# guangkun0818/speech2text

Hardware: AMD Instinct MI355X
Metric: audio-seconds/sec (train step, zipformer pruned-RNN-T) (higher is better)
Workload: dtype f32; 1 GPU; C3 zipformer pruned-RNN-T train step: chunk_size -1, 500 BPE, prune_range 5 (fbank+fwd+bwd+allreduce+ScaledAdam); accumulate_grad_batches=1, gemm_arith=bf16x2/3, per_gpu_batch=64, global_batch=64, labels_per_utt=50, parallelism=dp1

## Files before the change

include/s2t_mi355.h:

```cpp
#ifndef S2T_MI355_H_
#define S2T_MI355_H_

#ifdef __cplusplus
extern "C" {
#endif

int s2t_fbank_f32(const float* pcm, long pcm_stride, const long* num_samples, int batch,
                  const float* window400, const float* twiddle512, const int* mel_off,
                  const int* mel_k0, const float* mel_w, int nnz, int num_mel, float eps,
                  float scale_in, const float* cmvn_mean, const float* cmvn_istd, float* out,
                  int max_frames, long* out_frames, void* stream);

#define S2T_CTC_MAX_LABELS 1023
long s2t_ctc_workspace_floats(int B, int T, int Umax);
int s2t_ctc_loss_fwd_bwd(const float* logits, const long* targets, long tgt_stride,
                         const long* in_len, const long* tgt_len, int B, int T, int V, int Umax,
                         int blank, int zero_infinity, const float* grad_scale, float* workspace,
                         float* loss_per_utt, float* grad_logits, void* stream);

int s2t_fill_f32(float* p, long n, float v, void* stream);
int s2t_rnnt_row_exp(const float* x, long rows, int C, float* probs, float* rowmax, void* stream);
int s2t_rnnt_simple_pxpy(const float* am, const float* lm, const float* am_max,
                         const float* lm_max, const float* nrm, const long* symbols,
                         const long* boundary, int B, int S, int T, int C, int blank, float* px,
// ... 42 lines not shown
                        const float* bypass_scale, const float* g, const float* fm, int B, long rows, int D,
                        float* dx, float* d_orig, float* d_bypass_scale, float* dbias, float* dls,
                        void* stream);
int s2t_biasnorm_bwd(const float* x, const float* bias, const float* scales, const float* g,
                     long rows, int D, float* dx, float* dbias, float* dls, void* stream);
long s2t_balancer_bwd_workspace_floats(void);
int s2t_balancer_bwd(const float* x, long ldx, const float* g, long ldg, long rows, int C,
                     float min_mean, float max_mean, float min_rms, float max_rms,
                     float grad_scale, float* out, long ldo, float* workspace, int parity,
                     float act_off, void* stream);
int s2t_balancer_stats(const float* x, long ldx, long rows, int C, float* stats, void* stream);
int s2t_balancer_apply(const float* x, long ldx, const float* g, long ldg, long rows, int C,
                       float min_mean, float max_mean, float min_rms, float max_rms,
                       float grad_scale, float* out, long ldo, const float* stats, float act_off,
                       void* stream);


int s2t_zipconv_fwd(const float* u, long ld, int gate_off, const unsigned char* mask, int T, int B,
                    int C, int K, int chunk, const float* wc, const float* bc, const float* wk,
                    const float* bk, const float* scale, float* y, void* stream);
int s2t_zipconv_fwd_act(const float* u, long ld, int gate_off, const unsigned char* mask, int T, int B,
                        int C, int K, int chunk, const float* wc, const float* bc, const float* wk,
                        const float* bk, const float* scale, float* y, float* y_act, int act_kind,
                        void* stream);
int s2t_zipconv_bwd(const float* u, long ld, int gate_off, const unsigned char* mask, int T, int B,
                    int C, int K, int chunk, const float* wc, const float* wk, const float* bk,
                    const float* scale, const float* dy, float* du, float* dwc, float* dbc,
                    float* dwk, float* dbk, float* dscale, float* workspace, void* stream);
int s2t_zipconv_bwd_data(const float* u, long ld, int gate_off, const unsigned char* mask, int T,
                         int B, int C, int K, int chunk, const float* wc, const float* wk,
// ... 20 lines not shown
                        int delta_given, float* delta_ws, float* dqkp, float* dpos,
                        float* workspace, void* stream);
long s2t_relpos_attn_bwd_workspace_floats(int T, int B, int H, int pd);
int s2t_attn_apply(const float* W, const float* v, int T, int B, int H, int dv, int transpose,
                   float* out, void* stream);


long s2t_linear_wgrad_workspace_floats(int R, int N, int M);
int s2t_linear_wgrad(const float* g, long ldg, const float* a, long lda, int R, int N, int M,
                     float* dW, float* db, int accumulate, float* workspace, void* stream);

int s2t_whiten_metric(float* xtx, float* colsum, long n, int G, int cg, float* cov, float* mean,
                      float* scal, float* host_metric, float* workspace, void* stream);
int s2t_whiten_prep(const float* cov, const float* mean, const float* scal, int G, int cg, float* dcov,
                    float* bias, float* sums64, void* stream);
int s2t_gemm_x3p_sq(const float* A, long lda, const unsigned short* Bp, int N, int K, float* C, long ldc,
                    int M, const float* bias, const float* other, long ld_other, float* sums, int tile,
                    void* stream);
int s2t_sumsq64(const float* g, long numel, float* sums64, void* stream);
int s2t_whiten_combine64(const float* g, const float* pg, long numel, float grad_scale,
                         const float* sums64, float* out, void* stream);
int s2t_whiten_dcov(const float* cov, const float* mean, const float* scal, int G, int cg,
                    float* dcov, float* bias, float* sums, void* stream);
int s2t_whiten_apply(const float* g, const float* pg, long numel, float grad_scale, float* sums,
                     float* out, void* stream);
int s2t_limit_param_grad(const float* x, const float* g, float lo, float hi, long n, float* out,
                         void* stream);

int s2t_bestrq_labels(const float* feats, int B, int T, int F, const float* proj, int D,
                      const float* codebooks, int ncb, int K, int T2, long* labels, void* stream);
// ... 406 lines not shown
```

speech2text_amd/csrc/gemm_x3p.hip:

```cpp
#include "common.h"
#include "../../include/s2t_mi355.h"
#include <hip/hip_ext.h>
#include <algorithm>
#include <cstdint>
#include <cstdlib>
#include <utility>
#include <vector>

namespace {

typedef float f32x16 __attribute__((ext_vector_type(16)));
typedef float f32x2 __attribute__((ext_vector_type(2)));
typedef __bf16 bf16x2 __attribute__((ext_vector_type(2)));
typedef __bf16 bf16x8 __attribute__((ext_vector_type(8)));
typedef float f32x4 __attribute__((ext_vector_type(4)));
typedef unsigned u32x4 __attribute__((ext_vector_type(4)));
typedef const __attribute__((address_space(1))) float* gf32p;
typedef const __attribute__((address_space(1))) f32x4* gf32x4p;
typedef const __attribute__((address_space(1))) u32x4* gu32x4p;

__device__ __forceinline__ void split_pair(float x0, float x1, unsigned& p0, unsigned& p1,
                                           unsigned& p2) {
  f32x2 x = {x0, x1};
  p0 = __builtin_bit_cast(unsigned, __builtin_convertvector(x, bf16x2));
  f32x2 h = {__uint_as_float(p0 << 16), __uint_as_float(p0 & 0xFFFF0000u)};
  x = x - h;
  p1 = __builtin_bit_cast(unsigned, __builtin_convertvector(x, bf16x2));
  f32x2 h1 = {__uint_as_float(p1 << 16), __uint_as_float(p1 & 0xFFFF0000u)};
  x = x - h1;
  p2 = __builtin_bit_cast(unsigned, __builtin_convertvector(x, bf16x2));
}
__device__ __forceinline__ void split8(const f32x4 v0, const f32x4 v1, u32x4& q0, u32x4& q1,
                                       u32x4& q2) {
  unsigned a0, a1, a2, b0, b1, b2, c0, c1, c2, d0, d1, d2;
  split_pair(v0.x, v0.y, a0, a1, a2);
  split_pair(v0.z, v0.w, b0, b1, b2);
  split_pair(v1.x, v1.y, c0, c1, c2);
  split_pair(v1.z, v1.w, d0, d1, d2);
  q0 = u32x4{a0, b0, c0, d0};
  q1 = u32x4{a1, b1, c1, d1};
  q2 = u32x4{a2, b2, c2, d2};
}

__device__ __forceinline__ void split_pair2(float x0, float x1, unsigned& p0, unsigned& p1) {
  f32x2 x = {x0, x1};
  p0 = __builtin_bit_cast(unsigned, __builtin_convertvector(x, bf16x2));
// ... 138 lines not shown
__device__ __forceinline__ BalQ x3p_epi_balcoef(const X3P& g, int j, int n0, int wcb, int lane) {
  BalQ r;
  r.a = r.b = f32x4{0.f, 0.f, 0.f, 0.f};
  const int col = n0 + 32 * (wcb + j) + (lane & 7) * 4;
  if (col >= g.N) return r;
  r.a = *reinterpret_cast<const f32x4*>(g.bal_stats + 2048 + col);
  r.b = *reinterpret_cast<const f32x4*>(g.bal_stats + 3072 + col);
  return r;
}

__global__ __launch_bounds__(256) void bal_coef_kernel(const float* __restrict__ stats, float* __restrict__ coef,
                                                        int N, float n, float min_mean, float max_mean,
                                                        float min_rms, float max_rms, float gs) {
  const int c = blockIdx.x * 256 + threadIdx.x;
  if (c >= N) return;
  const float inv_n = 1.f / n;
  const float mean = stats[c] * inv_n, uvar = stats[1024 + c] * inv_n;
  const float raw_var = uvar - mean * mean;
  const bool live_v = raw_var > 1.0e-20f, live_r = uvar > 1.0e-20f;
  const float var = fmaxf(raw_var, 1.0e-20f);
  const float sd = sqrtf(var);
  const float rms = sqrtf(fmaxf(uvar, 1.0e-20f));
  const float m = mean / sd;
  const float mc = fminf(fmaxf(m, min_mean), max_mean);
  const float s_m = (m > mc) ? 1.f : ((m < mc) ? -1.f : 0.f);
  const float rc = fminf(fmaxf(rms, min_rms), max_rms);
  const float lq = logf(rc / rms);
  const float s_r = (lq > 0.f) ? -1.f : ((lq < 0.f) ? 1.f : 0.f);
  const float a = s_m * inv_n * (live_v ? (1.f / sd + mean * mean / (sd * var)) : 1.f / sd);
  const float b = (live_v ? -s_m * inv_n * mean / (sd * var) : 0.f) + (live_r ? s_r * inv_n / (rms * rms) : 0.f);
  const float lg_rms = fmaxf(sqrtf(fmaxf(a * a + 2.f * a * b * mean + b * b * uvar, 0.f)), 1.0e-20f);
  const float k = gs / lg_rms;
  coef[c] = a * k;
  coef[1024 + c] = b * k;
}

template <bool BAL = false>
__device__ __forceinline__ void x3p_epi_xform(const X3P& g, f32x16& a, float* scr, const EpiOps& o,
                                              const f32x4 bq, int h, int lane, const BalQ& bal = BalQ{}) {
  const int hi = lane >> 5, lo = lane & 31;
  const int er = lane >> 3, ec = (lane & 7) * 4;
#pragma unroll
  for (int r = 0; r < 8; ++r) scr[((r & 3) + 8 * (r >> 2) + 4 * hi) * 36 + lo] = a[8 * h + r];
  __builtin_amdgcn_fence(__ATOMIC_RELEASE, "workgroup", "local");
  __builtin_amdgcn_wave_barrier();
#pragma unroll
  for (int q = 0; q < 2; ++q) {
    f32x4 v = *reinterpret_cast<const f32x4*>(scr + (er + 8 * q) * 36 + ec);
    v += bq;
// ... 463 lines not shown
}

__global__ __launch_bounds__(256) void x3p_split_kernel(const float* __restrict__ base,
                                                        const S2tPlaneDesc* __restrict__ tab, int n,
                                                        unsigned short* __restrict__ dst) {
  int lo_d = 0, hi_d = n - 1;
  while (lo_d < hi_d) {
    const int mid = (lo_d + hi_d + 1) >> 1;
    if (tab[mid].blk_begin <= blockIdx.x) lo_d = mid; else hi_d = mid - 1;
  }
  const S2tPlaneDesc d = tab[lo_d];
  const int NT = (d.N + 31) >> 5, KB = 2 * ((d.K + 31) >> 5);
  const long q = (long)(blockIdx.x - d.blk_begin) * 4 + (threadIdx.x >> 6);
  if (q >= (long)NT * KB) return;
  const int nt = (int)(q / KB), kb = (int)(q - (long)nt * KB);
  const int lane = threadIdx.x & 63, lo = lane & 31, hi = lane >> 5;
  const int nn = 32 * nt + lo, k0 = 16 * kb + 8 * hi;
  const float* src = base + d.src_off;
  float v[8];
#pragma unroll
  for (int e = 0; e < 8; ++e) {
    const int k = k0 + e;
    const bool ok = nn < d.N && k < d.K;
    const long a = d.transposed ? (long)(ok ? k : 0) * d.ld + (ok ? nn : 0)
                                : (long)(ok ? nn : 0) * d.ld + (ok ? k : 0);
    const float x = src[a];
    v[e] = ok ? x : 0.f;
  }
  uint4 q0, q1, q2;
  split_pair(v[0], v[1], q0.x, q1.x, q2.x);
  split_pair(v[2], v[3], q0.y, q1.y, q2.y);
  split_pair(v[4], v[5], q0.z, q1.z, q2.z);
  split_pair(v[6], v[7], q0.w, q1.w, q2.w);
  unsigned short* o = dst + d.dst_off + (((long)nt * KB + kb) * 3 * 64 + lane) * 8;
  *reinterpret_cast<uint4*>(o) = q0;
  *reinterpret_cast<uint4*>(o + 512) = q1;
  *reinterpret_cast<uint4*>(o + 1024) = q2;
}

#define X3P_LAUNCH(KERNEL, GRID, BLOCK, SMEM)                                                     \
  do {                                                                                            \
    if (s2t_prof_start) {                                                                         \
      hipExtLaunchKernelGGL(KERNEL, dim3(GRID), dim3(BLOCK), SMEM, st, s2t_prof_start,            \
                            s2t_prof_stop, 0, g);                                                 \
      s2t_prof_start = s2t_prof_stop = nullptr;                                                   \
    } else {                                                                                      \
      hipLaunchKernelGGL(KERNEL, dim3(GRID), dim3(BLOCK), SMEM, st, g);                           \
    }                                                                                             \
  } while (0)

template <int TM, int TN, int WPC, int NP = 3, int KS = 1>
void launch_x3p_dma(X3P& g, hipStream_t st) {
// ... 404 lines not shown
```

speech2text_amd/csrc/whiten.hip:

```cpp
#include "common.h"
#include <algorithm>
#include <cstdint>

namespace {

constexpr int NT = 1024;

__device__ __forceinline__ float block_sum(float v, float* s_tmp) {
  v = wave_sum(v);
  const int lane = threadIdx.x & 63, wave = threadIdx.x >> 6;
  __syncthreads();
  if (lane == 0) s_tmp[wave] = v;
  __syncthreads();
  float t = (threadIdx.x < (NT >> 6)) ? s_tmp[threadIdx.x] : 0.f;
  if (wave == 0) {
    t = wave_sum(t);
    if (lane == 0) s_tmp[0] = t;
  }
  __syncthreads();
  return s_tmp[0];
}

__global__ __launch_bounds__(256) void whiten_metric_kernel(float* __restrict__ xtx,
                                                            float* __restrict__ colsum, float n,
// ... 101 lines not shown
    dcov[(long)ci * C + cj] = v;
    acc = fmaf(mean[cj], v, acc);
  }
  acc = wave_sum(acc);
  if ((threadIdx.x & 63) == 0) s_red[threadIdx.x >> 6] = acc;
  __syncthreads();
  if (threadIdx.x == 0) {
    bias[ci] = -((s_red[0] + s_red[1]) + (s_red[2] + s_red[3]));
    if (ci == 0) {
      sums[0] = 0.f;
      sums[1] = 0.f;
    }
  }
}

__global__ __launch_bounds__(256) void sumsq2_kernel(const float* __restrict__ a,
                                                     const float* __restrict__ b, long n,
                                                     float* __restrict__ sums) {
  __shared__ float s_a[4], s_b[4];
  float sa = 0.f, sb = 0.f;
  const long n4 = n >> 2;
  const float4* a4 = reinterpret_cast<const float4*>(a);
  const float4* b4 = reinterpret_cast<const float4*>(b);
  for (long e = (long)blockIdx.x * 256 + threadIdx.x; e < n4; e += (long)gridDim.x * 256) {
    const float4 x = a4[e], y = b4[e];
    sa += x.x * x.x + x.y * x.y + x.z * x.z + x.w * x.w;
    sb += y.x * y.x + y.y * y.y + y.z * y.z + y.w * y.w;
  }
  if (blockIdx.x == 0)
    for (long e = (n4 << 2) + threadIdx.x; e < n; e += 256) {
// ... 87 lines not shown
                     mean, scal, G, cg, dcov, bias, sums);
  S2T_CHECK_LAUNCH();
  return 0;
}

extern "C" int s2t_whiten_prep(const float* cov, const float* mean, const float* scal, int G, int cg,
                               float* dcov, float* bias, float* sums64, void* stream) {
  if (G <= 0 || cg <= 0 || !sums64) return -1;
  if (hipMemsetAsync(sums64, 0, 128 * sizeof(float), (hipStream_t)stream) != hipSuccess) return -3;
  hipLaunchKernelGGL(whiten_dcov_kernel, dim3(G * cg), dim3(256), 0, (hipStream_t)stream, cov, mean,
                     scal, G, cg, dcov, bias, sums64);
  S2T_CHECK_LAUNCH();
  return 0;
}

namespace {
__global__ __launch_bounds__(256) void sumsq64_kernel(const float* __restrict__ g, long numel,
                                                      float* __restrict__ sums64) {
  const long n4 = numel >> 2;
  const long stride = (long)gridDim.x * blockDim.x;
  const float4* g4 = reinterpret_cast<const float4*>(g);
  float acc = 0.f;
  for (long i = (long)blockIdx.x * blockDim.x + threadIdx.x; i < n4; i += stride) {
    const float4 v = g4[i];
    acc += (v.x * v.x + v.y * v.y) + (v.z * v.z + v.w * v.w);
  }
  for (long i = (n4 << 2) + (long)blockIdx.x * blockDim.x + threadIdx.x; i < numel; i += stride) acc += g[i] * g[i];
  acc = wave_sum(acc);
  if ((threadIdx.x & 63) == 0) atomicAdd(sums64 + ((blockIdx.x * 4 + (threadIdx.x >> 6)) & 63), acc);
}
// ... 67 lines not shown
```

speech2text_amd/csrc/zip_elem.hip:

```cpp
#include "common.h"
#include <algorithm>
#include <stdlib.h>

namespace {

__device__ __forceinline__ float log1p_fast(float e) {
  const float u = 1.f + e;
  return u == 1.f ? e : __logf(u) * __fdividef(e, u - 1.f);
}

__device__ __forceinline__ float swoosh_f(float x, float off, float c) {
  const float z = x - off;
  return fmaxf(z, 0.f) + log1p_fast(__expf(-fabsf(z))) - 0.08f * x - c;
}
__device__ __forceinline__ float swoosh_d(float x, float off) {
  return __fdividef(1.f, 1.f + __expf(off - x)) - 0.08f;
}

__global__ __launch_bounds__(256) void swoosh_fwd_kernel(const float* __restrict__ x,
                                                         float* __restrict__ y, long n, float off,
                                                         float c) {
  const long n4 = n >> 2;
  const long stride = (long)gridDim.x * blockDim.x;
  const float4* x4 = reinterpret_cast<const float4*>(x);
// ... 491 lines not shown
  __syncthreads();
  if (threadIdx.x < C) {
    const int c = threadIdx.x;
    const float* f0 = reinterpret_cast<const float*>(&sh[0][0][0]);
    const float* f1 = reinterpret_cast<const float*>(&sh[1][0][0]);
    atomicAdd(&sum[c], (f0[c] + f0[32 + c]) + (f0[64 + c] + f0[96 + c]));
    atomicAdd(&sumsq[c], (f1[c] + f1[32 + c]) + (f1[64 + c] + f1[96 + c]));
  }
}

__global__ __launch_bounds__(256) void balancer_apply_small_kernel(
    const float* __restrict__ x, const float* __restrict__ g, const float* __restrict__ stats,
    float* __restrict__ stats_next, float n, float min_mean, float max_mean, float min_rms, float max_rms,
    float grad_scale, long nquads, int C, float* __restrict__ out, float act_off) {
  __shared__ __attribute__((aligned(16))) float s_a[32], s_b[32];
  const float inv_n = 1.f / n;
  if (threadIdx.x < C) {
    const int c = threadIdx.x;
    const float mean = stats[c] * inv_n, uvar = stats[1024 + c] * inv_n;
    const float raw_var = uvar - mean * mean;
    const bool live_v = raw_var > 1.0e-20f, live_r = uvar > 1.0e-20f;
    const float var = fmaxf(raw_var, 1.0e-20f);
    const float sd = sqrtf(var);
    const float rms = sqrtf(fmaxf(uvar, 1.0e-20f));
    const float m = mean / sd;
    const float mc = fminf(fmaxf(m, min_mean), max_mean);
    const float s_m = (m > mc) ? 1.f : ((m < mc) ? -1.f : 0.f);
    const float rc = fminf(fmaxf(rms, min_rms), max_rms);
    const float lq = logf(rc / rms);
    const float s_r = (lq > 0.f) ? -1.f : ((lq < 0.f) ? 1.f : 0.f);
    const float a = s_m * inv_n * (live_v ? (1.f / sd + mean * mean / (sd * var)) : 1.f / sd);
    const float b = (live_v ? -s_m * inv_n * mean / (sd * var) : 0.f) +
                    (live_r ? s_r * inv_n / (rms * rms) : 0.f);
    const float lg_rms =
        fmaxf(sqrtf(fmaxf(a * a + 2.f * a * b * mean + b * b * uvar, 0.f)), 1.0e-20f);
    const float coef = grad_scale / lg_rms;
    s_a[c] = a * coef;
    s_b[c] = b * coef;
  }
  if (blockIdx.x == 0 && stats_next != nullptr)
    for (int c = threadIdx.x; c < 2 * 1024; c += 256) stats_next[c] = 0.f;
  __syncthreads();
  const int cq = C >> 2;
  const float4 a4 = *reinterpret_cast<const float4*>(&s_a[4 * (threadIdx.x & (cq - 1))]);
  const float4 b4 = *reinterpret_cast<const float4*>(&s_b[4 * (threadIdx.x & (cq - 1))]);
  const float4* x4 = reinterpret_cast<const float4*>(x);
  const float4* g4 = reinterpret_cast<const float4*>(g);
  float4* o4 = reinterpret_cast<float4*>(out);
  const long step = (long)gridDim.x * 256;
  for (long i = (long)blockIdx.x * 256 + threadIdx.x; i < nquads; i += 2 * step) {
    const bool two = i + step < nquads;
    float4 xv[2], gv[2];
    xv[0] = x4[i];
// ... 12 lines not shown
      }
      o4[i + u * step] = make_float4(gg.x + fabsf(gg.x) * fmaf(b4.x, xv[u].x, a4.x),
                                     gg.y + fabsf(gg.y) * fmaf(b4.y, xv[u].y, a4.y),
                                     gg.z + fabsf(gg.z) * fmaf(b4.z, xv[u].z, a4.z),
                                     gg.w + fabsf(gg.w) * fmaf(b4.w, xv[u].w, a4.w));
    }
  }
}

__global__ __launch_bounds__(256) void balancer_apply_fused_kernel(
    const float* __restrict__ x, long ldx, const float* __restrict__ g, long ldg,
    const float* __restrict__ stats, float* __restrict__ stats_next, float n, float min_mean,
    float max_mean, float min_rms, float max_rms, float grad_scale, long rows, int C,
    float* __restrict__ out, long ldo, float act_off) {
  __shared__ float s_a[1024], s_b[1024];
  const float inv_n = 1.f / n;
  for (int c = threadIdx.x; c < C; c += 256) {
    const float mean = stats[c] * inv_n, uvar = stats[1024 + c] * inv_n;
    const float raw_var = uvar - mean * mean;
    const bool live_v = raw_var > 1.0e-20f, live_r = uvar > 1.0e-20f;
    const float var = fmaxf(raw_var, 1.0e-20f);
    const float sd = sqrtf(var);
    const float rms = sqrtf(fmaxf(uvar, 1.0e-20f));
    const float m = mean / sd;
    const float mc = fminf(fmaxf(m, min_mean), max_mean);
    const float s_m = (m > mc) ? 1.f : ((m < mc) ? -1.f : 0.f);
    const float rc = fminf(fmaxf(rms, min_rms), max_rms);
    const float lq = logf(rc / rms);
    const float s_r = (lq > 0.f) ? -1.f : ((lq < 0.f) ? 1.f : 0.f);
    const float a = s_m * inv_n * (live_v ? (1.f / sd + mean * mean / (sd * var)) : 1.f / sd);
    const float b = (live_v ? -s_m * inv_n * mean / (sd * var) : 0.f) +
                    (live_r ? s_r * inv_n / (rms * rms) : 0.f);
    const float lg_rms =
        fmaxf(sqrtf(fmaxf(a * a + 2.f * a * b * mean + b * b * uvar, 0.f)), 1.0e-20f);
    const float coef = grad_scale / lg_rms;
    s_a[c] = a * coef;
    s_b[c] = b * coef;
  }
  if (blockIdx.x == 0 && stats_next != nullptr)
    for (int c = threadIdx.x; c < 2 * 1024; c += 256) stats_next[c] = 0.f;
  __syncthreads();
  const int tx = threadIdx.x & 63, ty = threadIdx.x >> 6;
  const long step = (long)gridDim.x * 4;
  for (int c0 = 0; c0 < C; c0 += 64) {
    const int c = c0 + tx;
    if (c >= C) continue;
    const float a = s_a[c], b = s_b[c];
    long r = (long)blockIdx.x * 4 + ty;
    for (; r + 3 * step < rows; r += 4 * step) {
      float gv[4], xv[4];
#pragma unroll
      for (int u = 0; u < 4; ++u) {
        gv[u] = g[(r + u * step) * ldg + c];
        xv[u] = x[(r + u * step) * ldx + c];
      }
#pragma unroll
      for (int u = 0; u < 4; ++u) {
        if (act_off >= 0.f) gv[u] *= swoosh_d(xv[u], act_off);
        out[(r + u * step) * ldo + c] = gv[u] + fabsf(gv[u]) * fmaf(b, xv[u], a);
      }
    }
    for (; r < rows; r += step) {
// ... 239 lines not shown
  if (bal_small(C, x, ldx, g, ldg, out, ldo)) {
    const long nq = rows * C / 4;
    hipLaunchKernelGGL(balancer_apply_small_kernel, dim3(bal_small_grid(nq)), dim3(256), 0, (hipStream_t)stream,
                       x, g, stats, (float*)nullptr, (float)rows, min_mean, max_mean, min_rms, max_rms, grad_scale,
                       nq, C, out, act_off);
    S2T_CHECK_LAUNCH();
    return 0;
  }
  hipLaunchKernelGGL(balancer_apply_fused_kernel, dim3((unsigned)std::min<long>((rows + 15) / 16, 2048)),
                     dim3(256), 0, (hipStream_t)stream, x, ldx, g, ldg, stats, (float*)nullptr,
                     (float)rows, min_mean, max_mean, min_rms, max_rms, grad_scale, rows, C, out, ldo,
                     act_off);
  S2T_CHECK_LAUNCH();
  return 0;
}
```

Baseline: 17950 audio-seconds/sec.

## Fuse balancer stats with coefficient computation and add one-pass whiten finish kernel

Adds a balancer stats kernel that reduces column sums with a last-block ticket and computes the per-channel balancer coefficients in the same launch, so the apply kernel only reads precomputed coefficients. Adds a whiten_finish kernel that builds the covariance, reduces the metric, computes the bias and splits the whitening matrix into bf16x3 pieces in one launch instead of several. Shared helpers (coefficient math, x3p fragment split) move into headers. The new entry points are only used if the Python side calls them, which is not shown, and the ticket-based grid reduction adds cross-block synchronization risk.

After: 17560 audio-seconds/sec. -2.1%, worse.

```diff
diff --git a/include/s2t_mi355.h b/include/s2t_mi355.h
--- a/include/s2t_mi355.h
+++ b/include/s2t_mi355.h
@@ -80,6 +80,12 @@
                        float min_mean, float max_mean, float min_rms, float max_rms,
                        float grad_scale, float* out, long ldo, const float* stats, float act_off,
                        void* stream);
+long s2t_balancer_stats_ws_floats(void);
+int s2t_balancer_stats_coef(const float* x, long ldx, long rows, int C, float min_mean, float max_mean,
+                            float min_rms, float max_rms, float grad_scale, float* stats, float* workspace,
+                            void* stream);
+int s2t_balancer_apply_coef(const float* x, long ldx, const float* g, long ldg, long rows, int C, float* out,
+                            long ldo, const float* stats, float act_off, void* stream);
 
 
 int s2t_zipconv_fwd(const float* u, long ld, int gate_off, const unsigned char* mask, int T, int B,
@@ -130,6 +136,9 @@
                       float* scal, float* host_metric, float* workspace, void* stream);
 int s2t_whiten_prep(const float* cov, const float* mean, const float* scal, int G, int cg, float* dcov,
                     float* bias, float* sums64, void* stream);
+int s2t_whiten_finish(float* xtx, float* colsum, long n, int G, int cg, float* cov, float* mean, float* scal,
+                      float* host_metric, float* workspace, float* bias, float* sums64, const void* tab,
+                      unsigned short* pieces, void* stream);
 int s2t_gemm_x3p_sq(const float* A, long lda, const unsigned short* Bp, int N, int K, float* C, long ldc,
                     int M, const float* bias, const float* other, long ld_other, float* sums, int tile,
                     void* stream);
diff --git a/speech2text_amd/csrc/balancer_coef.h b/speech2text_amd/csrc/balancer_coef.h
--- /dev/null
+++ b/speech2text_amd/csrc/balancer_coef.h
@@ -0,0 +1,26 @@
+#pragma once
+#include <hip/hip_runtime.h>
+
+__device__ __forceinline__ void s2t_bal_coef_of(float sum, float sumsq, float n, float min_mean, float max_mean,
+                                                float min_rms, float max_rms, float gs, float& ak, float& bk) {
+#pragma clang fp contract(off)
+  const float inv_n = 1.f / n;
+  const float mean = sum * inv_n, uvar = sumsq * inv_n;
+  const float raw_var = uvar - mean * mean;
+  const bool live_v = raw_var > 1.0e-20f, live_r = uvar > 1.0e-20f;
+  const float var = fmaxf(raw_var, 1.0e-20f);
+  const float sd = sqrtf(var);
+  const float rms = sqrtf(fmaxf(uvar, 1.0e-20f));
+  const float m = mean / sd;
+  const float mc = fminf(fmaxf(m, min_mean), max_mean);
+  const float s_m = (m > mc) ? 1.f : ((m < mc) ? -1.f : 0.f);
+  const float rc = fminf(fmaxf(rms, min_rms), max_rms);
+  const float lq = logf(rc / rms);
+  const float s_r = (lq > 0.f) ? -1.f : ((lq < 0.f) ? 1.f : 0.f);
+  const float a = s_m * inv_n * (live_v ? (1.f / sd + mean * mean / (sd * var)) : 1.f / sd);
+  const float b = (live_v ? -s_m * inv_n * mean / (sd * var) : 0.f) + (live_r ? s_r * inv_n / (rms * rms) : 0.f);
+  const float lg_rms = fmaxf(sqrtf(fmaxf(a * a + 2.f * a * b * mean + b * b * uvar, 0.f)), 1.0e-20f);
+  const float k = gs / lg_rms;
+  ak = a * k;
+  bk = b * k;
+}
diff --git a/speech2text_amd/csrc/gemm_x3p.hip b/speech2text_amd/csrc/gemm_x3p.hip
--- a/speech2text_amd/csrc/gemm_x3p.hip
+++ b/speech2text_amd/csrc/gemm_x3p.hip
@@ -1,5 +1,7 @@
 #include "common.h"
 #include "../../include/s2t_mi355.h"
+#include "x3p_split.h"
+#include "balancer_coef.h"
 #include <hip/hip_ext.h>
 #include <algorithm>
 #include <cstdint>
@@ -19,17 +21,6 @@
 typedef const __attribute__((address_space(1))) f32x4* gf32x4p;
 typedef const __attribute__((address_space(1))) u32x4* gu32x4p;
 
-__device__ __forceinline__ void split_pair(float x0, float x1, unsigned& p0, unsigned& p1,
-                                           unsigned& p2) {
-  f32x2 x = {x0, x1};
-  p0 = __builtin_bit_cast(unsigned, __builtin_convertvector(x, bf16x2));
-  f32x2 h = {__uint_as_float(p0 << 16), __uint_as_float(p0 & 0xFFFF0000u)};
-  x = x - h;
-  p1 = __builtin_bit_cast(unsigned, __builtin_convertvector(x, bf16x2));
-  f32x2 h1 = {__uint_as_float(p1 << 16), __uint_as_float(p1 & 0xFFFF0000u)};
-  x = x - h1;
-  p2 = __builtin_bit_cast(unsigned, __builtin_convertvector(x, bf16x2));
-}
 __device__ __forceinline__ void split8(const f32x4 v0, const f32x4 v1, u32x4& q0, u32x4& q1,
                                        u32x4& q2) {
   unsigned a0, a1, a2, b0, b1, b2, c0, c1, c2, d0, d1, d2;
@@ -198,25 +189,7 @@
                                                         float min_rms, float max_rms, float gs) {
   const int c = blockIdx.x * 256 + threadIdx.x;
   if (c >= N) return;
-  const float inv_n = 1.f / n;
-  const float mean = stats[c] * inv_n, uvar = stats[1024 + c] * inv_n;
-  const float raw_var = uvar - mean * mean;
-  const bool live_v = raw_var > 1.0e-20f, live_r = uvar > 1.0e-20f;
-  const float var = fmaxf(raw_var, 1.0e-20f);
-  const float sd = sqrtf(var);
-  const float rms = sqrtf(fmaxf(uvar, 1.0e-20f));
-  const float m = mean / sd;
-  const float mc = fminf(fmaxf(m, min_mean), max_mean);
-  const float s_m = (m > mc) ? 1.f : ((m < mc) ? -1.f : 0.f);
-  const float rc = fminf(fmaxf(rms, min_rms), max_rms);
-  const float lq = logf(rc / rms);
-  const float s_r = (lq > 0.f) ? -1.f : ((lq < 0.f) ? 1.f : 0.f);
-  const float a = s_m * inv_n * (live_v ? (1.f / sd + mean * mean / (sd * var)) : 1.f / sd);
-  const float b = (live_v ? -s_m * inv_n * mean / (sd * var) : 0.f) + (live_r ? s_r * inv_n / (rms * rms) : 0.f);
-  const float lg_rms = fmaxf(sqrtf(fmaxf(a * a + 2.f * a * b * mean + b * b * uvar, 0.f)), 1.0e-20f);
-  const float k = gs / lg_rms;
-  coef[c] = a * k;
-  coef[1024 + c] = b * k;
+  s2t_bal_coef_of(stats[c], stats[1024 + c], n, min_mean, max_mean, min_rms, max_rms, gs, coef[c], coef[1024 + c]);
 }
 
 template <bool BAL = false>
@@ -710,28 +683,10 @@
   const long q = (long)(blockIdx.x - d.blk_begin) * 4 + (threadIdx.x >> 6);
   if (q >= (long)NT * KB) return;
   const int nt = (int)(q / KB), kb = (int)(q - (long)nt * KB);
-  const int lane = threadIdx.x & 63, lo = lane & 31, hi = lane >> 5;
-  const int nn = 32 * nt + lo, k0 = 16 * kb + 8 * hi;
   const float* src = base + d.src_off;
-  float v[8];
-#pragma unroll
-  for (int e = 0; e < 8; ++e) {
-    const int k = k0 + e;
-    const bool ok = nn < d.N && k < d.K;
-    const long a = d.transposed ? (long)(ok ? k : 0) * d.ld + (ok ? nn : 0)
-                                : (long)(ok ? nn : 0) * d.ld + (ok ? k : 0);
-    const float x = src[a];
-    v[e] = ok ? x : 0.f;
-  }
-  uint4 q0, q1, q2;
-  split_pair(v[0], v[1], q0.x, q1.x, q2.x);
-  split_pair(v[2], v[3], q0.y, q1.y, q2.y);
-  split_pair(v[4], v[5], q0.z, q1.z, q2.z);
-  split_pair(v[6], v[7], q0.w, q1.w, q2.w);
-  unsigned short* o = dst + d.dst_off + (((long)nt * KB + kb) * 3 * 64 + lane) * 8;
-  *reinterpret_cast<uint4*>(o) = q0;
-  *reinterpret_cast<uint4*>(o + 512) = q1;
-  *reinterpret_cast<uint4*>(o + 1024) = q2;
+  x3p_split_fragment(d.N, d.K, nt, kb, threadIdx.x & 63, dst + d.dst_off, [&](int nn, int k) {
+    return src[d.transposed ? (long)k * d.ld + nn : (long)nn * d.ld + k];
+  });
 }
 
 #define X3P_LAUNCH(KERNEL, GRID, BLOCK, SMEM)                                                     \
diff --git a/speech2text_amd/csrc/whiten.hip b/speech2text_amd/csrc/whiten.hip
--- a/speech2text_amd/csrc/whiten.hip
+++ b/speech2text_amd/csrc/whiten.hip
@@ -1,4 +1,5 @@
 #include "common.h"
+#include "x3p_split.h"
 #include <algorithm>
 #include <cstdint>
 
@@ -139,6 +140,155 @@
   }
 }
 
+__device__ __forceinline__ void xw_store(float* p, float v) {
+  __hip_atomic_store(p, v, __ATOMIC_RELAXED, __HIP_MEMORY_SCOPE_AGENT);
+}
+__device__ __forceinline__ float xw_load(const float* p) {
+  return __hip_atomic_load(p, __ATOMIC_RELAXED, __HIP_MEMORY_SCOPE_AGENT);
+}
+__device__ __forceinline__ void xw_stores_done() { asm volatile("s_waitcnt vmcnt(0)" ::: "memory"); }
+__global__ __launch_bounds__(1024) void whiten_finish_kernel(float* __restrict__ xtx, float* __restrict__ colsum,
+                                                             float n, int G, int cg, float* cov,
+                                                             float* __restrict__ mean, float* __restrict__ scal,
+                                                             float* host_metric, float* __restrict__ ws,
+                                                             float* __restrict__ bias, float* __restrict__ sums64,
+                                                             const S2tPlaneDesc* __restrict__ desc,
+                                                             unsigned short* __restrict__ pieces) {
+  __shared__ float s_red[2][4];
+  __shared__ unsigned s_old;
+  __shared__ float s_sc[4];
+  __shared__ float s_mean[1024];
+  const int C = G * cg;
+  const int ci = blockIdx.x;
+  const int g = ci / cg, i = ci - g * cg;
+  const float inv_n = 1.f / n;
+  float dsum = 0.f, sq = 0.f;
+  float* xrow = xtx + (long)ci * C;
+  if (threadIdx.x < 256) {
+    const float mi = colsum[ci] * inv_n;
+    for (int j = threadIdx.x; j < cg; j += 256) {
+      const int cj = g * cg + j;
+      if ((cj >> 6) < (ci >> 6)) continue;
+      const float v = xrow[cj] - mi * colsum[cj];
+      xw_store(cov + ((long)g * cg + i) * cg + j, v);
+      sq = fmaf(v, v, sq);
+      if (i == j) dsum = v;
+      if ((cj >> 6) > (ci >> 6)) {
+        xw_store(cov + ((long)g * cg + j) * cg + i, v);
+        sq = fmaf(v, v, sq);
+      }
+    }
+    xw_stores_done();
+  }
+  __syncthreads();
+  for (int j = threadIdx.x; j < C; j += 1024) xrow[j] = 0.f;
+  if (threadIdx.x < 256) {
+    dsum = wave_sum(dsum);
+    sq = wave_sum(sq);
+    if ((threadIdx.x & 63) == 0) {
+      s_red[0][threadIdx.x >> 6] = dsum;
+      s_red[1][threadIdx.x >> 6] = sq;
+    }
+  }
+  __syncthreads();
+  unsigned* ticket = reinterpret_cast<unsigned*>(ws);
+  float* part = ws + 4;
+  if (threadIdx.x == 0) {
+    xw_store(part + 2 * ci, (s_red[0][0] + s_red[0][1]) + (s_red[0][2] + s_red[0][3]));
+    xw_store(part + 2 * ci + 1, (s_red[1][0] + s_red[1][1]) + (s_red[1][2] + s_red[1][3]));
+    xw_stores_done();
+    s_old = atomicAdd(ticket, 1u);
+  }
+  __syncthreads();
+  if (s_old != gridDim.x - 1) return;
+  __builtin_amdgcn_fence(__ATOMIC_ACQUIRE, "agent");
+  if (threadIdx.x < 256) {
+    dsum = 0.f;
+    sq = 0.f;
+    for (int r = threadIdx.x; r < C; r += 256) {
+      dsum += xw_load(part + 2 * r);
+      sq += xw_load(part + 2 * r + 1);
+      const float m = colsum[r] * inv_n;
+      mean[r] = m;
+      s_mean[r] = m;
+    }
+    dsum = wave_sum(dsum);
+    sq = wave_sum(sq);
+  }
+  __syncthreads();
+  if (threadIdx.x < 256 && (threadIdx.x & 63) == 0) {
+    s_red[0][threadIdx.x >> 6] = dsum;
+    s_red[1][threadIdx.x >> 6] = sq;
+  }
+  __syncthreads();
+  for (int r = threadIdx.x; r < C; r += 1024) colsum[r] = 0.f;
+  if (threadIdx.x == 0) {
+    const float dtot = (s_red[0][0] + s_red[0][1]) + (s_red[0][2] + s_red[0][3]);
+    const float sqtot = (s_red[1][0] + s_red[1][1]) + (s_red[1][2] + s_red[1][3]);
+    const float md = dtot / (float)C;
+    const float covsq = sqtot / (float)C;
+    const float denom = md * md + 1.0e-20f;
+    const float metric = covsq / denom;
+    scal[0] = md;
+    scal[1] = covsq;
+    scal[2] = denom;
+    scal[3] = metric;
+    s_sc[0] = md;
+    s_sc[1] = covsq;
+    s_sc[2] = denom;
+    *ticket = 0u;
+    if (host_metric)
+      __hip_atomic_store(host_metric, metric, __ATOMIC_RELAXED, __HIP_MEMORY_SCOPE_SYSTEM);
+  }
+  if (pieces == nullptr) return;
+  if (threadIdx.x < 128) sums64[threadIdx.x] = 0.f;
+  __syncthreads();
+  const float md = s_sc[0], covsq = s_sc[1], denom = s_sc[2];
+  const float k = 4.f / (float)C;
+  const float a = 1.f / denom, d = covsq * md / (denom * denom);
+  const int lane = threadIdx.x & 63, wave = threadIdx.x >> 6;
+#pragma unroll 4
+  for (int r = wave; r < C; r += 16) {
+    const int gr = r / cg;
+    const float* crow = cov + (long)r * cg - (long)gr * cg;
+    float acc[4] = {0.f, 0.f, 0.f, 0.f};
+    const int lo = gr * cg, hi = lo + cg;
+    for (int base = (lo >> 8) << 8; base < hi; base += 256) {
+#pragma unroll
+      for (int w = 0; w < 4; ++w) {
+        const int cj = base + 64 * w + lane;
+        if (cj >= lo && cj < hi) {
+          float v = crow[cj] * a;
+          if (r == cj) v -= d;
+          v *= k;
+          acc[w] = fmaf(s_mean[cj], v, acc[w]);
+        }
+      }
+    }
+#pragma unroll
+    for (int w = 0; w < 4; ++w) acc[w] = wave_sum(acc[w]);
+    if (lane == 0) bias[r] = -((acc[0] + acc[1]) + (acc[2] + acc[3]));
+  }
+  const S2tPlaneDesc ds = desc[0];
+  const int KB = x3p_frag_kb(ds.K);
+  const int nfrag = x3p_frag_nt(ds.N) * KB;
+#pragma unroll 2
+  for (int f = wave; f < nfrag; f += 16) {
+    const int nt = f / KB, kb = f - nt * KB;
+    x3p_split_fragment(ds.N, ds.K, nt, kb, lane, pieces + ds.dst_off, [&](int nn, int kk) {
+      const int r = ds.transposed ? kk : nn, c = ds.transposed ? nn : kk;
+      const int gr = r / cg;
+      float v = 0.f;
+      if (c / cg == gr) {
+        v = cov[(long)r * cg + (c - gr * cg)] * a;
+        if (r == c) v -= d;
+        v *= k;
+      }
+      return v;
+    });
+  }
+}
+
 __global__ __launch_bounds__(256) void sumsq2_kernel(const float* __restrict__ a,
                                                      const float* __restrict__ b, long n,
                                                      float* __restrict__ sums) {
@@ -256,6 +406,18 @@
   return 0;
 }
 
+extern "C" int s2t_whiten_finish(float* xtx, float* colsum, long n, int G, int cg, float* cov, float* mean,
+                                 float* scal, float* host_metric, float* workspace, float* bias,
+                                 float* sums64, const void* tab, unsigned short* pieces, void* stream) {
+  if (G <= 0 || cg <= 0 || n <= 0 || !workspace || (long)G * cg > 1024) return -1;
+  if (pieces && (!bias || !sums64 || !tab || (reinterpret_cast<uintptr_t>(pieces) & 15))) return -1;
+  hipLaunchKernelGGL(whiten_finish_kernel, dim3(G * cg), dim3(1024), 0, (hipStream_t)stream, xtx, colsum,
+                     (float)n, G, cg, cov, mean, scal, host_metric, workspace, bias, sums64,
+                     reinterpret_cast<const S2tPlaneDesc*>(tab), pieces);
+  S2T_CHECK_LAUNCH();
+  return 0;
+}
+
 namespace {
 __global__ __launch_bounds__(256) void sumsq64_kernel(const float* __restrict__ g, long numel,
                                                       float* __restrict__ sums64) {
diff --git a/speech2text_amd/csrc/x3p_split.h b/speech2text_amd/csrc/x3p_split.h
--- /dev/null
+++ b/speech2text_amd/csrc/x3p_split.h
@@ -0,0 +1,50 @@
+#pragma once
+#include "../../include/s2t_mi355.h"
+#include "common.h"
+
+namespace {
+
+typedef float x3ps_f32x2 __attribute__((ext_vector_type(2)));
+typedef __bf16 x3ps_bf16x2 __attribute__((ext_vector_type(2)));
+
+__device__ __forceinline__ void split_pair(float x0, float x1, unsigned& p0, unsigned& p1,
+                                           unsigned& p2) {
+  x3ps_f32x2 x = {x0, x1};
+  p0 = __builtin_bit_cast(unsigned, __builtin_convertvector(x, x3ps_bf16x2));
+  x3ps_f32x2 h = {__uint_as_float(p0 << 16), __uint_as_float(p0 & 0xFFFF0000u)};
+  x = x - h;
+  p1 = __builtin_bit_cast(unsigned, __builtin_convertvector(x, x3ps_bf16x2));
+  x3ps_f32x2 h1 = {__uint_as_float(p1 << 16), __uint_as_float(p1 & 0xFFFF0000u)};
+  x = x - h1;
+  p2 = __builtin_bit_cast(unsigned, __builtin_convertvector(x, x3ps_bf16x2));
+}
+
+__device__ __forceinline__ int x3p_frag_kb(int K) { return 2 * ((K + 31) >> 5); }
+__device__ __forceinline__ int x3p_frag_nt(int N) { return (N + 31) >> 5; }
+
+template <class Load>
+__device__ __forceinline__ void x3p_split_fragment(int N, int K, int nt, int kb, int lane,
+                                                   unsigned short* __restrict__ plane, Load&& load) {
+  const int KB = x3p_frag_kb(K);
+  const int lo = lane & 31, hi = lane >> 5;
+  const int nn = 32 * nt + lo, k0 = 16 * kb + 8 * hi;
+  float v[8];
+#pragma unroll
+  for (int e = 0; e < 8; ++e) {
+    const int k = k0 + e;
+    const bool ok = nn < N && k < K;
+    const float x = load(ok ? nn : 0, ok ? k : 0);
+    v[e] = ok ? x : 0.f;
+  }
+  uint4 q0, q1, q2;
+  split_pair(v[0], v[1], q0.x, q1.x, q2.x);
+  split_pair(v[2], v[3], q0.y, q1.y, q2.y);
+  split_pair(v[4], v[5], q0.z, q1.z, q2.z);
+  split_pair(v[6], v[7], q0.w, q1.w, q2.w);
+  unsigned short* o = plane + (((long)nt * KB + kb) * 3 * 64 + lane) * 8;
+  *reinterpret_cast<uint4*>(o) = q0;
+  *reinterpret_cast<uint4*>(o + 512) = q1;
+  *reinterpret_cast<uint4*>(o + 1024) = q2;
+}
+
+}
diff --git a/speech2text_amd/csrc/zip_elem.hip b/speech2text_amd/csrc/zip_elem.hip
--- a/speech2text_amd/csrc/zip_elem.hip
+++ b/speech2text_amd/csrc/zip_elem.hip
@@ -1,5 +1,8 @@
 #include "common.h"
+#include "balancer_coef.h"
 #include <algorithm>
+#include <cstdint>
+#include <mutex>
 #include <stdlib.h>
 
 namespace {
@@ -529,29 +532,9 @@
     float* __restrict__ stats_next, float n, float min_mean, float max_mean, float min_rms, float max_rms,
     float grad_scale, long nquads, int C, float* __restrict__ out, float act_off) {
   __shared__ __attribute__((aligned(16))) float s_a[32], s_b[32];
-  const float inv_n = 1.f / n;
   if (threadIdx.x < C) {
     const int c = threadIdx.x;
-    const float mean = stats[c] * inv_n, uvar = stats[1024 + c] * inv_n;
-    const float raw_var = uvar - mean * mean;
-    const bool live_v = raw_var > 1.0e-20f, live_r = uvar > 1.0e-20f;
-    const float var = fmaxf(raw_var, 1.0e-20f);
-    const float sd = sqrtf(var);
-    const float rms = sqrtf(fmaxf(uvar, 1.0e-20f));
-    const float m = mean / sd;
-    const float mc = fminf(fmaxf(m, min_mean), max_mean);
-    const float s_m = (m > mc) ? 1.f : ((m < mc) ? -1.f : 0.f);
-    const float rc = fminf(fmaxf(rms, min_rms), max_rms);
-    const float lq = logf(rc / rms);
-    const float s_r = (lq > 0.f) ? -1.f : ((lq < 0.f) ? 1.f : 0.f);
-    const float a = s_m * inv_n * (live_v ? (1.f / sd + mean * mean / (sd * var)) : 1.f / sd);
-    const float b = (live_v ? -s_m * inv_n * mean / (sd * var) : 0.f) +
-                    (live_r ? s_r * inv_n / (rms * rms) : 0.f);
-    const float lg_rms =
-        fmaxf(sqrtf(fmaxf(a * a + 2.f * a * b * mean + b * b * uvar, 0.f)), 1.0e-20f);
-    const float coef = grad_scale / lg_rms;
-    s_a[c] = a * coef;
-    s_b[c] = b * coef;
+    s2t_bal_coef_of(stats[c], stats[1024 + c], n, min_mean, max_mean, min_rms, max_rms, grad_scale, s_a[c], s_b[c]);
   }
   if (blockIdx.x == 0 && stats_next != nullptr)
     for (int c = threadIdx.x; c < 2 * 1024; c += 256) stats_next[c] = 0.f;
@@ -594,29 +577,8 @@
     float max_mean, float min_rms, float max_rms, float grad_scale, long rows, int C,
     float* __restrict__ out, long ldo, float act_off) {
   __shared__ float s_a[1024], s_b[1024];
-  const float inv_n = 1.f / n;
-  for (int c = threadIdx.x; c < C; c += 256) {
-    const float mean = stats[c] * inv_n, uvar = stats[1024 + c] * inv_n;
-    const float raw_var = uvar - mean * mean;
-    const bool live_v = raw_var > 1.0e-20f, live_r = uvar > 1.0e-20f;
-    const float var = fmaxf(raw_var, 1.0e-20f);
-    const float sd = sqrtf(var);
-    const float rms = sqrtf(fmaxf(uvar, 1.0e-20f));
-    const float m = mean / sd;
-    const float mc = fminf(fmaxf(m, min_mean), max_mean);
-    const float s_m = (m > mc) ? 1.f : ((m < mc) ? -1.f : 0.f);
-    const float rc = fminf(fmaxf(rms, min_rms), max_rms);
-    const float lq = logf(rc / rms);
-    const float s_r = (lq > 0.f) ? -1.f : ((lq < 0.f) ? 1.f : 0.f);
-    const float a = s_m * inv_n * (live_v ? (1.f / sd + mean * mean / (sd * var)) : 1.f / sd);
-    const float b = (live_v ? -s_m * inv_n * mean / (sd * var) : 0.f) +
-                    (live_r ? s_r * inv_n / (rms * rms) : 0.f);
-    const float lg_rms =
-        fmaxf(sqrtf(fmaxf(a * a + 2.f * a * b * mean + b * b * uvar, 0.f)), 1.0e-20f);
-    const float coef = grad_scale / lg_rms;
-    s_a[c] = a * coef;
-    s_b[c] = b * coef;
-  }
+  for (int c = threadIdx.x; c < C; c += 256)
+    s2t_bal_coef_of(stats[c], stats[1024 + c], n, min_mean, max_mean, min_rms, max_rms, grad_scale, s_a[c], s_b[c]);
   if (blockIdx.x == 0 && stats_next != nullptr)
     for (int c = threadIdx.x; c < 2 * 1024; c += 256) stats_next[c] = 0.f;
   __syncthreads();
@@ -626,6 +588,287 @@
     const int c = c0 + tx;
     if (c >= C) continue;
     const float a = s_a[c], b = s_b[c];
+    long r = (long)blockIdx.x * 4 + ty;
+    for (; r + 3 * step < rows; r += 4 * step) {
+      float gv[4], xv[4];
+#pragma unroll
+      for (int u = 0; u < 4; ++u) {
+        gv[u] = g[(r + u * step) * ldg + c];
+        xv[u] = x[(r + u * step) * ldx + c];
+      }
+#pragma unroll
+      for (int u = 0; u < 4; ++u) {
+        if (act_off >= 0.f) gv[u] *= swoosh_d(xv[u], act_off);
+        out[(r + u * step) * ldo + c] = gv[u] + fabsf(gv[u]) * fmaf(b, xv[u], a);
+      }
+    }
+    for (; r < rows; r += step) {
+      const float xs = x[r * ldx + c];
+      float gv = g[r * ldg + c];
+      if (act_off >= 0.f) gv *= swoosh_d(xs, act_off);
+      out[r * ldo + c] = gv + fabsf(gv) * fmaf(b, xs, a);
+    }
+  }
+}
+
+
+__device__ __forceinline__ void part_store(float* p, float v) {
+  __hip_atomic_store(p, v, __ATOMIC_RELAXED, __HIP_MEMORY_SCOPE_AGENT);
+}
+__device__ __forceinline__ float part_load(const float* p) {
+  return __hip_atomic_load(p, __ATOMIC_RELAXED, __HIP_MEMORY_SCOPE_AGENT);
+}
+__device__ __forceinline__ void stores_done() { asm volatile("s_waitcnt vmcnt(0)" ::: "memory"); }
+
+struct BalCoefArgs {
+  float n, min_mean, max_mean, min_rms, max_rms, gs;
+};
+
+__global__ __launch_bounds__(256) void col_stats_ticket_kernel(const float* __restrict__ x, long rows, int C,
+                                                               long ld, float* __restrict__ stats,
+                                                               float* part, unsigned* ticket,
+                                                               BalCoefArgs k) {
+  const int c = blockIdx.y * 64 + threadIdx.x;
+  const int Cp = gridDim.y * 64;
+  float s = 0.f, q = 0.f;
+  if (c < C) {
+    const long step = (long)gridDim.x * 4;
+    long r = (long)blockIdx.x * 4 + threadIdx.y;
+    for (; r + 7 * step < rows; r += 8 * step) {
+      float v[8];
+#pragma unroll
+      for (int u = 0; u < 8; ++u) v[u] = x[(r + u * step) * ld + c];
+#pragma unroll
+      for (int u = 0; u < 8; ++u) {
+        s += v[u];
+        q = fmaf(v[u], v[u], q);
+      }
+    }
+    for (; r < rows; r += step) {
+      const float v = x[r * ld + c];
+      s += v;
+      q = fmaf(v, v, q);
+    }
+  }
+  __shared__ float sh[2][4][64];
+  __shared__ unsigned s_old;
+  sh[0][threadIdx.y][threadIdx.x] = s;
+  sh[1][threadIdx.y][threadIdx.x] = q;
+  __syncthreads();
+  if (threadIdx.y == 0) {
+    s = sh[0][0][threadIdx.x] + sh[0][1][threadIdx.x] + sh[0][2][threadIdx.x] + sh[0][3][threadIdx.x];
+    q = sh[1][0][threadIdx.x] + sh[1][1][threadIdx.x] + sh[1][2][threadIdx.x] + sh[1][3][threadIdx.x];
+    float* p = part + (long)blockIdx.x * 2 * Cp;
+    part_store(p + c, s);
+    part_store(p + Cp + c, q);
+    stores_done();
+  }
+  __syncthreads();
+  if (threadIdx.x == 0 && threadIdx.y == 0) s_old = atomicAdd(ticket + blockIdx.y, 1u);
+  __syncthreads();
+  if (s_old != gridDim.x - 1) return;
+  s = 0.f;
+  q = 0.f;
+  {
+    const int nb = (int)gridDim.x;
+    int b = threadIdx.y;
+    for (; b + 124 < nb; b += 128) {
+      float v[32], w[32];
+#pragma unroll
+      for (int u = 0; u < 32; ++u) {
+        v[u] = part_load(part + (long)(b + 4 * u) * 2 * Cp + c);
+        w[u] = part_load(part + (long)(b + 4 * u) * 2 * Cp + Cp + c);
+      }
+#pragma unroll
+      for (int u = 0; u < 32; ++u) {
+        s += v[u];
+        q += w[u];
+      }
+    }
+    for (; b + 28 < nb; b += 32) {
+      float v[8], w[8];
+#pragma unroll
+      for (int u = 0; u < 8; ++u) {
+        v[u] = part_load(part + (long)(b + 4 * u) * 2 * Cp + c);
+        w[u] = part_load(part + (long)(b + 4 * u) * 2 * Cp + Cp + c);
+      }
+#pragma unroll
+      for (int u = 0; u < 8; ++u) {
+        s += v[u];
+        q += w[u];
+      }
+    }
+    for (; b < nb; b += 4) {
+      s += part_load(part + (long)b * 2 * Cp + c);
+      q += part_load(part + (long)b * 2 * Cp + Cp + c);
+    }
+  }
+  __syncthreads();
+  sh[0][threadIdx.y][threadIdx.x] = s;
+  sh[1][threadIdx.y][threadIdx.x] = q;
+  __syncthreads();
+  if (threadIdx.y == 0 && c < C) {
+    s = sh[0][0][threadIdx.x] + sh[0][1][threadIdx.x] + sh[0][2][threadIdx.x] + sh[0][3][threadIdx.x];
+    q = sh[1][0][threadIdx.x] + sh[1][1][threadIdx.x] + sh[1][2][threadIdx.x] + sh[1][3][threadIdx.x];
+    stats[c] = s;
+    stats[1024 + c] = q;
+    float ak, bk;
+    s2t_bal_coef_of(s, q, k.n, k.min_mean, k.max_mean, k.min_rms, k.max_rms, k.gs, ak, bk);
+    stats[2048 + c] = ak;
+    stats[3072 + c] = bk;
+  }
+  if (threadIdx.x == 0 && threadIdx.y == 0) ticket[blockIdx.y] = 0u;
+}
+
+__global__ __launch_bounds__(256) void col_stats_small_ticket_kernel(const float* __restrict__ x, long nquads,
+                                                                     int C, float* __restrict__ stats,
+                                                                     float* part, unsigned* ticket,
+                                                                     BalCoefArgs k) {
+  const int cq = C >> 2;
+  float4 s = make_float4(0.f, 0.f, 0.f, 0.f), q = s;
+  const float4* x4 = reinterpret_cast<const float4*>(x);
+  const long step = (long)gridDim.x * 256;
+  long i = (long)blockIdx.x * 256 + threadIdx.x;
+  for (; i + 3 * step < nquads; i += 4 * step) {
+    float4 v[4];
+#pragma unroll
+    for (int u = 0; u < 4; ++u) v[u] = x4[i + u * step];
+#pragma unroll
+    for (int u = 0; u < 4; ++u) {
+      s.x += v[u].x; s.y += v[u].y; s.z += v[u].z; s.w += v[u].w;
+      q.x = fmaf(v[u].x, v[u].x, q.x); q.y = fmaf(v[u].y, v[u].y, q.y);
+      q.z = fmaf(v[u].z, v[u].z, q.z); q.w = fmaf(v[u].w, v[u].w, q.w);
+    }
+  }
+  for (; i < nquads; i += step) {
+    const float4 v = x4[i];
+    s.x += v.x; s.y += v.y; s.z += v.z; s.w += v.w;
+    q.x = fmaf(v.x, v.x, q.x); q.y = fmaf(v.y, v.y, q.y); q.z = fmaf(v.z, v.z, q.z); q.w = fmaf(v.w, v.w, q.w);
+  }
+  __shared__ float4 sh[2][4][8];
+  __shared__ unsigned s_old;
+  const int lane = threadIdx.x & 63, wave = threadIdx.x >> 6;
+  const float* f0 = reinterpret_cast<const float*>(&sh[0][0][0]);
+  const float* f1 = reinterpret_cast<const float*>(&sh[1][0][0]);
+#pragma unroll
+  for (int o = 32; o >= 1; o >>= 1) {
+    if (o >= cq) {
+      s.x += __shfl_xor(s.x, o, 64); s.y += __shfl_xor(s.y, o, 64);
+      s.z += __shfl_xor(s.z, o, 64); s.w += __shfl_xor(s.w, o, 64);
+      q.x += __shfl_xor(q.x, o, 64); q.y += __shfl_xor(q.y, o, 64);
+      q.z += __shfl_xor(q.z, o, 64); q.w += __shfl_xor(q.w, o, 64);
+    }
+  }
+  if (lane < cq) {
+    sh[0][wave][lane] = s;
+    sh[1][wave][lane] = q;
+  }
+  __syncthreads();
+  float* psum = part;
+  float* psq = part + (long)gridDim.x * C;
+  if (threadIdx.x < C) {
+    const int c = threadIdx.x;
+    part_store(psum + (long)blockIdx.x * C + c, (f0[c] + f0[32 + c]) + (f0[64 + c] + f0[96 + c]));
+    part_store(psq + (long)blockIdx.x * C + c, (f1[c] + f1[32 + c]) + (f1[64 + c] + f1[96 + c]));
+    stores_done();
+  }
+  __syncthreads();
+  if (threadIdx.x == 0) s_old = atomicAdd(ticket, 1u);
+  __syncthreads();
+  if (s_old != gridDim.x - 1) return;
+  float ts = 0.f, tq = 0.f;
+  const long pn = (long)gridDim.x * C;
+  long j = threadIdx.x;
+  for (; j + 7 * 256 < pn; j += 8 * 256) {
+    float v[8], w[8];
+#pragma unroll
+    for (int u = 0; u < 8; ++u) {
+      v[u] = part_load(psum + j + u * 256);
+      w[u] = part_load(psq + j + u * 256);
+    }
+#pragma unroll
+    for (int u = 0; u < 8; ++u) {
+      ts += v[u];
+      tq += w[u];
+    }
+  }
+  for (; j < pn; j += 256) {
+    ts += part_load(psum + j);
+    tq += part_load(psq + j);
+  }
+#pragma unroll
+  for (int o = 32; o >= 4; o >>= 1) {
+    if (o >= C) {
+      ts += __shfl_xor(ts, o, 64);
+      tq += __shfl_xor(tq, o, 64);
+    }
+  }
+  __syncthreads();
+  float* r0 = reinterpret_cast<float*>(&sh[0][0][0]);
+  float* r1 = reinterpret_cast<float*>(&sh[1][0][0]);
+  if (lane < C) {
+    r0[32 * wave + lane] = ts;
+    r1[32 * wave + lane] = tq;
+  }
+  __syncthreads();
+  if (threadIdx.x < C) {
+    const int c = threadIdx.x;
+    ts = (r0[c] + r0[32 + c]) + (r0[64 + c] + r0[96 + c]);
+    tq = (r1[c] + r1[32 + c]) + (r1[64 + c] + r1[96 + c]);
+    stats[c] = ts;
+    stats[1024 + c] = tq;
+    float ak, bk;
+    s2t_bal_coef_of(ts, tq, k.n, k.min_mean, k.max_mean, k.min_rms, k.max_rms, k.gs, ak, bk);
+    stats[2048 + c] = ak;
+    stats[3072 + c] = bk;
+  }
+  if (threadIdx.x == 0) *ticket = 0u;
+}
+
+__global__ __launch_bounds__(256) void balancer_apply_coef_small_kernel(
+    const float* __restrict__ x, const float* __restrict__ g, const float* __restrict__ coef, long nquads, int C,
+    float* __restrict__ out, float act_off) {
+  const int cq = C >> 2;
+  const float4 a4 = *reinterpret_cast<const float4*>(coef + 4 * (threadIdx.x & (cq - 1)));
+  const float4 b4 = *reinterpret_cast<const float4*>(coef + 1024 + 4 * (threadIdx.x & (cq - 1)));
+  const float4* x4 = reinterpret_cast<const float4*>(x);
+  const float4* g4 = reinterpret_cast<const float4*>(g);
+  float4* o4 = reinterpret_cast<float4*>(out);
+  const long step = (long)gridDim.x * 256;
+  for (long i = (long)blockIdx.x * 256 + threadIdx.x; i < nquads; i += 2 * step) {
+    const bool two = i + step < nquads;
+    float4 xv[2], gv[2];
+    xv[0] = x4[i];
+    gv[0] = g4[i];
+    xv[1] = x4[two ? i + step : i];
+    gv[1] = g4[two ? i + step : i];
+#pragma unroll
+    for (int u = 0; u < 2; ++u) {
+      if (u == 1 && !two) break;
+      float4 gg = gv[u];
+      if (act_off >= 0.f) {
+        gg.x *= swoosh_d(xv[u].x, act_off);
+        gg.y *= swoosh_d(xv[u].y, act_off);
+        gg.z *= swoosh_d(xv[u].z, act_off);
+        gg.w *= swoosh_d(xv[u].w, act_off);
+      }
+      o4[i + u * step] = make_float4(gg.x + fabsf(gg.x) * fmaf(b4.x, xv[u].x, a4.x),
+                                     gg.y + fabsf(gg.y) * fmaf(b4.y, xv[u].y, a4.y),
+                                     gg.z + fabsf(gg.z) * fmaf(b4.z, xv[u].z, a4.z),
+                                     gg.w + fabsf(gg.w) * fmaf(b4.w, xv[u].w, a4.w));
+    }
+  }
+}
+
+__global__ __launch_bounds__(256) void balancer_apply_coef_kernel(
+    const float* __restrict__ x, long ldx, const float* __restrict__ g, long ldg,
+    const float* __restrict__ coef, long rows, int C, float* __restrict__ out, long ldo, float act_off) {
+  const int tx = threadIdx.x & 63, ty = threadIdx.x >> 6;
+  const long step = (long)gridDim.x * 4;
+  for (int c0 = 0; c0 < C; c0 += 64) {
+    const int c = c0 + tx;
+    if (c >= C) continue;
+    const float a = coef[c], b = coef[1024 + c];
     long r = (long)blockIdx.x * 4 + ty;
     for (; r + 3 * step < rows; r += 4 * step) {
       float gv[4], xv[4];
@@ -895,3 +1138,71 @@
   S2T_CHECK_LAUNCH();
   return 0;
 }
+
+namespace {
+constexpr int kTicketSlots = 1024, kTicketWords = 16, kTicketDevs = 16;
+unsigned* g_tickets[kTicketDevs] = {};
+unsigned g_ticket_next[kTicketDevs] = {};
+std::mutex g_ticket_mu;
+unsigned* next_tickets() {
+  int dev = 0;
+  if (hipGetDevice(&dev) != hipSuccess || dev < 0 || dev >= kTicketDevs) return nullptr;
+  std::lock_guard<std::mutex> lock(g_ticket_mu);
+  if (!g_tickets[dev]) {
+    unsigned* p = nullptr;
+    const size_t bytes = (size_t)kTicketSlots * kTicketWords * sizeof(unsigned);
+    if (hipMalloc((void**)&p, bytes) != hipSuccess) return nullptr;
+    if (hipMemset(p, 0, bytes) != hipSuccess || hipDeviceSynchronize() != hipSuccess) {
+      (void)hipFree(p);
+      return nullptr;
+    }
+    g_tickets[dev] = p;
+  }
+  return g_tickets[dev] + (size_t)(g_ticket_next[dev]++ % kTicketSlots) * kTicketWords;
+}
+}
+
+extern "C" long s2t_balancer_stats_ws_floats(void) { return 2L * 256 * BAL_MAXC; }
+
+extern "C" int s2t_balancer_stats_coef(const float* x, long ldx, long rows, int C, float min_mean,
+                                       float max_mean, float min_rms, float max_rms, float grad_scale,
+                                       float* stats, float* workspace, void* stream) {
+  if (rows <= 0 || C <= 0) return 0;
+  if (C > BAL_MAXC || !stats || !workspace || (reinterpret_cast<uintptr_t>(workspace) & 15)) return -1;
+  unsigned* ticket = next_tickets();
+  if (!ticket) return -3;
+  const BalCoefArgs k{(float)rows, min_mean, max_mean, min_rms, max_rms, grad_scale};
+  if (bal_small(C, x, ldx, nullptr, 0, nullptr, 0)) {
+    const long nq = rows * C / 4;
+    hipLaunchKernelGGL(col_stats_small_ticket_kernel, dim3(bal_small_grid(nq)), dim3(256), 0, (hipStream_t)stream,
+                       x, nq, C, stats, workspace, ticket, k);
+    S2T_CHECK_LAUNCH();
+    return 0;
+  }
+  const int gy = (C + 63) / 64;
+  long gx = (rows + 4 * 16 - 1) / (4 * 16);
+  gx = gx > 256 ? 256 : (gx < 1 ? 1 : gx);
+  hipLaunchKernelGGL(col_stats_ticket_kernel, dim3((unsigned)gx, gy), dim3(64, 4), 0, (hipStream_t)stream, x,
+                     rows, C, ldx, stats, workspace, ticket, k);
+  S2T_CHECK_LAUNCH();
+  return 0;
+}
+
+extern "C" int s2t_balancer_apply_coef(const float* x, long ldx, const float* g, long ldg, long rows, int C,
+                                       float* out, long ldo, const float* stats, float act_off,
+                                       void* stream) {
+  if (rows <= 0 || C <= 0) return 0;
+  if (C > BAL_MAXC || !stats) return -1;
+  const float* coef = stats + 2 * BAL_MAXC;
+  if (bal_small(C, x, ldx, g, ldg, out, ldo) && (reinterpret_cast<uintptr_t>(coef) & 15) == 0) {
+    const long nq = rows * C / 4;
+    hipLaunchKernelGGL(balancer_apply_coef_small_kernel, dim3(bal_small_grid(nq)), dim3(256), 0,
+                       (hipStream_t)stream, x, g, coef, nq, C, out, act_off);
+    S2T_CHECK_LAUNCH();
+    return 0;
+  }
+  hipLaunchKernelGGL(balancer_apply_coef_kernel, dim3((unsigned)std::min<long>((rows + 15) / 16, 2048)),
+                     dim3(256), 0, (hipStream_t)stream, x, ldx, g, ldg, coef, rows, C, out, ldo, act_off);
+  S2T_CHECK_LAUNCH();
+  return 0;
+}
```
